# ansonb/RECON

Hardware: AMD Instinct MI355X
Metric: edges aggregated/sec (GAT fwd+bwd) on synthetic KG-context graphs (higher is better)
Workload: dtype f32

## Files before the change

recon_amd/csrc/gat_atp.hip:

```cpp
#include <math.h>
#include <stdlib.h>
#include "recon_common.h"

#include <type_traits>

namespace recon {
namespace {

constexpr int kBlock = 256;

__device__ __forceinline__ int xcd_block(int b, int nb) {
    const int q = nb >> 3, r = nb & 7, x = b & 7, i = b >> 3;
    return (x < r ? x * (q + 1) : r * (q + 1) + (x - r) * q) + i;
}
template <int VEC, bool B16>
__device__ __forceinline__ void load_in(float (&r)[VEC], const float* base, int64_t e) {
    if constexpr (!B16) {
        load_vec<VEC>(r, base + e);
    } else {
        const uint16_t* b = reinterpret_cast<const uint16_t*>(base) + e;
        if constexpr (VEC == 4) {
            const uint2 t = *reinterpret_cast<const uint2*>(b);
            r[0] = __builtin_bit_cast(float, t.x << 16); r[1] = __builtin_bit_cast(float, t.x & 0xffff0000u);
            r[2] = __builtin_bit_cast(float, t.y << 16); r[3] = __builtin_bit_cast(float, t.y & 0xffff0000u);
        } else if constexpr (VEC == 2) {
// ... 70 lines not shown
                                                       const float* __restrict__ gu, int32_t D, int32_t W, float* __restrict__ ga,
                                                       float* __restrict__ ga2, uint32_t* __restrict__ rezero, int32_t rezero_words) {
    __shared__ float red[256];
    const int d = blockIdx.x, h = blockIdx.y;
    if (rezero && d == 0 && h == 0)
        for (int i = threadIdx.x; i < rezero_words; i += 256) rezero[i] = 0u;
    const int64_t row = (static_cast<int64_t>(h) * D + d) * W;
    const float a2v = a2[h * D + d];
    float s = 0.f;
    for (int w = threadIdx.x; w < W; w += 256) {
        const float g = gu[static_cast<int64_t>(h) * W + w];
        s = fmaf(a[row + w], g, s);
        if (ga) ga[row + w] += a2v * g;
    }
    red[threadIdx.x] = s;
    __syncthreads();
    for (int off = 128; off > 0; off >>= 1) {
        if (threadIdx.x < off) red[threadIdx.x] += red[threadIdx.x + off];
        __syncthreads();
    }
    if (threadIdx.x == 0 && ga2) ga2[h * D + d] = red[0];
}

__global__ void __launch_bounds__(256) k_atp_weights_finish(const float* __restrict__ partial, int32_t splits, int32_t W, int32_t D, int32_t H,
                                                            const float* __restrict__ a, const float* __restrict__ a2,
                                                            const float* __restrict__ gu, float* __restrict__ ga, float* __restrict__ ga2,
                                                            uint32_t* __restrict__ rezero, int32_t rezero_words) {
    __shared__ float tile[32][33];
    if (rezero && blockIdx.x == 0)
        for (int i = threadIdx.x; i < rezero_words; i += 256) rezero[i] = 0u;
    const int tw = (W + 31) / 32, td = (D + 31) / 32, ntile = tw * td * H;
    if (static_cast<int>(blockIdx.x) < ntile) {
        const int b = blockIdx.x, h = b / (td * tw), m0 = ((b / td) % tw) * 32, n0 = (b % td) * 32;
        const int tx = threadIdx.x & 31, ty = threadIdx.x >> 5;
        const int64_t MN = static_cast<int64_t>(W) * D;
        const float* pz = partial + static_cast<int64_t>(h) * splits * MN;
        float acc[4] = {0.f, 0.f, 0.f, 0.f};
        int64_t off[4];
        bool ok[4];
#pragma unroll
        for (int i = 0; i < 4; ++i) {
            const int m = m0 + ty + 8 * i, n = n0 + tx;
            ok[i] = m < W && n < D;
            off[i] = ok[i] ? static_cast<int64_t>(m) * D + n : 0;
        }
        for (int z = 0; z < splits; ++z) {
#pragma unroll
            for (int i = 0; i < 4; ++i) acc[i] += pz[z * MN + off[i]];
        }
#pragma unroll
        for (int i = 0; i < 4; ++i) tile[ty + 8 * i][tx] = ok[i] ? acc[i] : 0.f;
        __syncthreads();
#pragma unroll
        for (int i = 0; i < 4; ++i) {
            const int n = n0 + ty + 8 * i, m = m0 + tx;
            if (m < W && n < D)
                ga[(static_cast<int64_t>(h) * D + n) * W + m] = fmaf(a2[h * D + n], gu[static_cast<int64_t>(h) * W + m], tile[tx][ty + 8 * i]);
        }
    } else if (ga2) {
        const int lane = threadIdx.x & 63, wave = threadIdx.x >> 6;
        const int r0 = (static_cast<int>(blockIdx.x) - ntile) * 8 + wave * 2;
#pragma unroll
        for (int i = 0; i < 2; ++i) {
            const int r = r0 + i;
            if (r >= H * D) break;
            const int h = r / D;
            float sum = 0.f;
            for (int w = 4 * lane; w < W; w += 256) {
                const float4 av = *reinterpret_cast<const float4*>(a + static_cast<int64_t>(r) * W + w);
                const float4 gv = *reinterpret_cast<const float4*>(gu + static_cast<int64_t>(h) * W + w);
                sum = fmaf(av.x, gv.x, fmaf(av.y, gv.y, fmaf(av.z, gv.z, fmaf(av.w, gv.w, sum))));
            }
#pragma unroll
            for (int off = 32; off > 0; off >>= 1) sum += __shfl_xor(sum, off, 64);
            if (lane == 0) ga2[r] = sum;
        }
    }
}

__global__ void __launch_bounds__(256) k_elu_grad_q(const float* __restrict__ gy, int32_t ld_gy, const float* __restrict__ y,
// ... 1458 lines not shown
}
template <int NJ, bool B16 = false>
__global__ void __launch_bounds__(256) k_skinny_tn_partial(const SkinnyJob j0, const SkinnyJob j1, const SkinnyJob j2) {
    __shared__ float red[NJ][256];
    const int which = static_cast<int>(blockIdx.x) < j0.nb ? 0 : (static_cast<int>(blockIdx.x) < j0.nb + j1.nb ? 1 : 2);
    const SkinnyJob& jb = which == 0 ? j0 : (which == 1 ? j1 : j2);
    skinny_block<NJ, B16, false>(jb, blockIdx.x - (which == 0 ? 0 : (which == 1 ? j0.nb : j0.nb + j1.nb)), red, nullptr, SkinnySrc{nullptr, nullptr, nullptr}, false);
}

template <int VEC, int KR, bool B16>
__global__ void __launch_bounds__(kBlock) k_gat_atp_src_skinny(const AtpSrcK p, int32_t nsrc, const SkinnyJob j0, const SkinnyJob j1, const SkinnyJob j2,
                                                               const SkinnySrc sr) {
    static_assert(kBlock == 256, "skinny_block: 4 waves");
    __shared__ float red[8][256];
    extern __shared__ __attribute__((aligned(16))) float gsl[];
    const int bx = blockIdx.x;
    if (bx < nsrc) { atp_src_wave<VEC, KR>(p, bx, nsrc); return; }
    const int b = bx - nsrc;
    const int which = b < j0.nb ? 0 : (b < j0.nb + j1.nb ? 1 : 2);
    const SkinnyJob& jb = which == 0 ? j0 : (which == 1 ? j1 : j2);
    skinny_block<8, B16, true>(jb, b - (which == 0 ? 0 : (which == 1 ? j0.nb : j0.nb + j1.nb)), red, gsl, sr, which == 1);
}

struct SkinnyRedJob { const float* partial; float* out; int64_t S1, S2; int32_t nb, nj, K, P, nblocks; };
__global__ void __launch_bounds__(1024) k_skinny_reduce(const SkinnyRedJob j0, const SkinnyRedJob j1, const SkinnyRedJob j2) {
    __shared__ float red[64][17];
    const int which = static_cast<int>(blockIdx.x) < j0.nblocks ? 0 : (static_cast<int>(blockIdx.x) < j0.nblocks + j1.nblocks ? 1 : 2);
    const SkinnyRedJob& jb = which == 0 ? j0 : (which == 1 ? j1 : j2);
    const float* __restrict__ partial = jb.partial;
    float* __restrict__ out = jb.out;
    const int nb = jb.nb, nj = jb.nj, K = jb.K, P = jb.P;
    const int64_t S1 = jb.S1, S2 = jb.S2;
    const int bid = blockIdx.x - (which == 0 ? 0 : (which == 1 ? j0.nblocks : j0.nblocks + j1.nblocks));
    const int e = threadIdx.x & 15, grp = threadIdx.x >> 4;
    const int idx = bid * 16 + e;
    const int tot = nj * K;
    const int per = (nb + 63) / 64;
    const int b0 = grp * per, b1 = min(nb, (grp + 1) * per);
    float s0 = 0.f, s1 = 0.f, s2 = 0.f, s3 = 0.f;
    if (idx < tot) {
        int b = b0;
        for (; b + 4 <= b1; b += 4) {
            s0 += partial[static_cast<int64_t>(b) * tot + idx];
            s1 += partial[static_cast<int64_t>(b + 1) * tot + idx];
            s2 += partial[static_cast<int64_t>(b + 2) * tot + idx];
            s3 += partial[static_cast<int64_t>(b + 3) * tot + idx];
        }
        for (; b < b1; ++b) s0 += partial[static_cast<int64_t>(b) * tot + idx];
    }
    red[grp][e] = (s0 + s1) + (s2 + s3);
    __syncthreads();
    if (grp == 0 && idx < tot) {
        float t = 0.f;
#pragma unroll
        for (int g = 0; g < 64; ++g) t += red[g][e];
        const int j = idx / K, c = idx % K;
        out[(j % P) * S1 + (j / P) * S2 + c] = t;
    }
}

struct AtpShape { int vec, kr, ht; };
bool atp_shape(int F, int R, int H, AtpShape* s) {
    const int mx = F > R ? F : R;
    int vec;
    if (F % 4 == 0 && R % 4 == 0) vec = 4;
    else if (F % 2 == 0 && R % 2 == 0) vec = 2;
    else return false;
    int kr = (mx + 64 * vec - 1) / (64 * vec);
    if (kr > 2 && kr <= 4) kr = 4; else if (kr > 4 && kr <= 8) kr = 8; else if (kr > 8) return false;
    int ht = 1;
    while (ht < H && ht < 8) ht <<= 1;
    while (ht > 1 && 2 * ht * kr * vec > 96) ht >>= 1;
    if (2 * ht * kr * vec > 96) return false;
    s->vec = vec; s->kr = kr; s->ht = ht;
    return true;
}
bool al(const void* p, size_t a) { return (reinterpret_cast<uintptr_t>(p) & (a - 1)) == 0; }
int atp_key(const AtpShape& s) { return s.vec * 1000 + s.kr * 10 + (s.ht == 8 ? 3 : s.ht == 4 ? 2 : s.ht == 2 ? 1 : 0); }

#define ATP_DISPATCH(S, CALL)                                                                              \
    do {                                                                                                   \
// ... 359 lines not shown
    int32_t ld_gh = b->ld_gout;
    const int64_t ld_ghp = bx3_kp(static_cast<int32_t>(HD));
    const bool gh_planes = hx2 || (b->gh_split && a->a_split && !(reinterpret_cast<uintptr_t>(b->gh_split) & 15) && (D % 8) == 0 &&
                                   ((b->ld_gout | a->ld_out) & 3) == 0);
    uint16_t* ghp = gh_planes ? static_cast<uint16_t*>(b->gh_split) : nullptr;
    const int64_t ldi = (static_cast<int64_t>(NR) + 7) / 8 * 8;
    const size_t inv_off = align_up(static_cast<size_t>(2) * N * bx3_kp(static_cast<int32_t>(HD)) * 2, 256);
    const bool row_scaled = hx2 && D <= 256 && ((a->ld_out | b->ld_gout) & 3) == 0 && cfg_char(CFG_ATP_ROW_SCALE) != '0' &&
                            inv_off + static_cast<size_t>(H) * ldi * sizeof(float) <= recon_gat_atp_bwd_split_bytes(N, D, H);
    float* row_inv = row_scaled ? reinterpret_cast<float*>(static_cast<char*>(b->gh_split) + inv_off) : nullptr;
    if (phases & RECON_ATP_BWD_PREPARE) {
        if (hx2 && !row_scaled) {
            rc = hx2_amax(b->grad_out, N, static_cast<int32_t>(HD), b->ld_gout, atp_q(a, 3), st);
            if (rc != RECON_OK) return rc;
        }
        hipLaunchKernelGGL(k_elu_grad_q, dim3(static_cast<unsigned>(ceil_div64(1LL * NR * H, 16))), dim3(256), 0, st, b->grad_out, b->ld_gout, a->out,
                           a->ld_out, NR, H, D, a->concat, ((a->concat || rw.row_node) && !hx2) ? b->g_h : nullptr, b->q, ghp, hx2 ? 2LL * D : ld_ghp,
                           hx2 ? static_cast<int64_t>(D) : static_cast<int64_t>(NR) * ld_ghp, hx2 ? 1 : 0,
                           hx2 ? atp_scale_g(a) : Hx2Scale{nullptr, nullptr, 1.f}, row_inv, ldi, row_scaled ? atp_q(a, 3) : nullptr, rw.row_node);
    }
    if (a->concat || rw.row_node) { gh = b->g_h; ld_gh = static_cast<int32_t>(HD); }
    GemmBatch bt;
    bt.batch = H; bt.epilogue = 0;
    if (phases & RECON_ATP_BWD_INPUTS) {
    {
        OperandDesc A = plain_operand(gh, ld_gh);
        OperandDesc B = plain_operand(a->a, W);
        OutputDesc C = plain_output(b->g_V, static_cast<int64_t>(H) * W);
        bt.a_bs = D; bt.b_bs = static_cast<int64_t>(D) * W; bt.c_bs = W;
        if (hx2)
            rc = gemm_hx2_batched(NR, W, D, b->gh_split, D, 2LL * D, 2LL * NR * D,
                                  static_cast<const char*>(a->a_split) + split_part_bytes(D, W, H), C, bt,
                                  row_scaled ? Hx2Scale{nullptr, nullptr, 1.f} : atp_scale_g(a), atp_scale_a(a), st, 0, row_inv, ldi);
        else if (a->a_split && bx3_supported(A, D, bt))
            rc = gemm_bx3_batched(NR, W, D, A, static_cast<const char*>(a->a_split) + split_part_bytes(D, W, H), C, bt, st);
        else
            rc = gemm_f32_batched(NR, W, D, A, true, B, false, C, bt, 1, nullptr, st);
        if (rc != RECON_OK) return rc;
    }
    {
        AtpBwdK p;
        p.rowptr = rw.rowptr; p.row_node = rw.row_node; p.src = g->src; p.eid = a->ee_index ? a->ee_index : g->eid;
        p.gee_by_slot = a->ee_index ? 1 : 0;
        p.gee_b16 = b->g_ee_bf16 ? 1 : 0;
        if (b->g_ee_bf16 && !(a->io_bf16 && !a->ee_index && b->g_edge_embed && recon_gat_atp_bwd_gee_bf16_supported(F, R, D, H))) return RECON_ERR_UNSUPPORTED;
        p.x = a->x; p.ee = a->edge_embed; p.keep = a->keep; p.sigma = a->sigma; p.Z = a->Z; p.Zk = a->Zk;
// ... 78 lines not shown
                    const Prod& q = pr[i];
                    if (q.rows <= 0) {
                        for (int j = 0; j < q.nj; ++j) (void)hipMemsetAsync(q.out + (j % q.P) * q.S1 + (j / q.P) * q.S2, 0, sizeof(float) * q.K, st);
                        continue;
                    }
                    const int rpb = skinny_rpb(q.rows);
                    const int nb = static_cast<int>(ceil_div64(q.rows, rpb));
                    float* part = b->partial2 + i * third;
                    sj[i] = SkinnyJob{q.G, q.X, q.gather, part, q.ldg, q.nj, q.rows, q.K, rpb, nb};
                    rj[i] = SkinnyRedJob{part, q.out, q.S1, q.S2, nb, q.nj, q.K, q.P, static_cast<int32_t>(ceil_div64(1LL * q.nj * q.K, 16))};
                    if (q.nj > nj_max) nj_max = q.nj;
                    nb_total += nb; nr_total += rj[i].nblocks;
                }
                if (share) { launch_src(); if (nb_total == 0) return; }
                else {
                    if (nb_total == 0) return;
                    const dim3 gp(static_cast<unsigned>(nb_total));
                    if (a->io_bf16) {
                        if (nj_max <= 8) hipLaunchKernelGGL((k_skinny_tn_partial<8, true>), gp, dim3(256), 0, st, sj[0], sj[1], sj[2]);
                        else hipLaunchKernelGGL((k_skinny_tn_partial<16, true>), gp, dim3(256), 0, st, sj[0], sj[1], sj[2]);
                    } else if (nj_max <= 8) hipLaunchKernelGGL((k_skinny_tn_partial<8>), gp, dim3(256), 0, st, sj[0], sj[1], sj[2]);
                    else hipLaunchKernelGGL((k_skinny_tn_partial<16>), gp, dim3(256), 0, st, sj[0], sj[1], sj[2]);
                }
                hipLaunchKernelGGL(k_skinny_reduce, dim3(static_cast<unsigned>(nr_total)), dim3(1024), 0, st, rj[0], rj[1], rj[2]);
            };
            if (H <= 8) {
                const Prod pr[3] = {{b->Gs, 2 * H, H, a->x, rw.row_node, NR, F, H, W, 0, b->g_u},
                                    {b->Gs + H, 2 * H, H, a->x, nullptr, N, F, H, W, 0, b->g_u + F},
                                    {b->g_sigma, H, H, a->edge_embed, ee_gather, E, R, H, W, 0, b->g_u + 2 * F}};
                run_jobs(pr, 3);
            } else {
                for (int j = 0; j < 2 * H; ++j) {
                    const Prod one = {b->Gs + j, 2 * H, 1, a->x, j < H ? rw.row_node : nullptr, j < H ? NR : N, F, 1, W, 0,
                                      b->g_u + static_cast<int64_t>(j % H) * W + (j / H) * F};
                    run_jobs(&one, 1);
                }
                for (int h0 = 0; h0 < H; h0 += 16) {
                    const int nh = H - h0 < 16 ? H - h0 : 16;
                    const Prod one = {b->g_sigma + h0, H, nh, a->edge_embed, ee_gather, E, R, nh, W, 0, b->g_u + static_cast<int64_t>(h0) * W + 2 * F};
                    run_jobs(&one, 1);
                }
            }
        }
        RECON_CHECK_LAUNCH();
    }
    }
    if (b->g_a || b->g_a_2) {
        if (!b->g_a) return RECON_ERR_INVALID;
        if (phases & RECON_ATP_BWD_WEIGHTS) {
            OperandDesc A = plain_operand(a->V, static_cast<int64_t>(H) * W);
            OperandDesc B = plain_operand(gh, ld_gh);
            OutputDesc C = plain_output(b->g_a, W);
            GemmBatch bw = bt;
            bw.a_bs = W; bw.b_bs = D; bw.c_bs = static_cast<int64_t>(D) * W; bw.c_transpose = 1;
            const int64_t ldv = static_cast<int64_t>(H) * W;
            if (hx2) {
                const int sk = bx3_kmajor_splits(NR, bx3_kmajor_split_k(W, D, NR, H));
                rc = gemm_hx2_kmajor_batched(W, D, NR, a->V, 2LL * W, W, 2LL * NR * W, b->gh_split, 2LL * D, D, 2LL * NR * D,
                                             H, sk, b->partial, static_cast<const char*>(a->aux) + kHx2ZeroPageOffset, atp_scale_v(a), atp_scale_g(a), st,
                                             atp_dst_shared(a), row_inv, ldi);
                if (rc == RECON_OK && (phases & RECON_ATP_BWD_EARLY_SUM)) rc = splitk_reduce(b->partial, sk, W, D, C, bw.c_bs, H, 0, true, st);
            } else if (gh_planes && bx3_kmajor_supported(a->V, ldv, W, ld_ghp, D, W, D)) {
                const int sk = bx3_kmajor_splits(NR, bx3_kmajor_split_k(W, D, NR, H));
                rc = gemm_bx3_kmajor_batched(W, D, NR, a->V, ldv, W, b->gh_split, ld_ghp, static_cast<int64_t>(NR) * ld_ghp, D, H, sk, b->partial, st);
                if (rc == RECON_OK) rc = splitk_reduce(b->partial, sk, W, D, C, bw.c_bs, H, 0, true, st);
            } else {
                const int sk = gemm_pick_split_k(W, D, NR, H);
                rc = gemm_f32_batched(W, D, NR, A, false, B, false, C, bw, sk, b->partial, st);
            }
            if (rc != RECON_OK) return rc;
        }
        if ((phases & RECON_ATP_BWD_FINISH) && hx2 && !(phases & RECON_ATP_BWD_EARLY_SUM)) {
            const int sk = bx3_kmajor_splits(NR, bx3_kmajor_split_k(W, D, NR, H));
            const int ntile = static_cast<int>(ceil_div64(W, 32) * ceil_div64(D, 32)) * H;
            hipLaunchKernelGGL(k_atp_weights_finish, dim3(static_cast<unsigned>(ntile + ceil_div64(1LL * H * D, 8))), dim3(256), 0, st, b->partial, sk, W,
                               D, H, a->a, a->a_2, b->g_u, b->g_a, b->g_a_2, atp_q(a, 3), kHx2QuantityWords);
        } else if (phases & RECON_ATP_BWD_FINISH)
        hipLaunchKernelGGL(k_score_vec_bwd, dim3(static_cast<unsigned>(D), static_cast<unsigned>(H)), dim3(256), 0, st, a->a, a->a_2, b->g_u,
                           D, W, b->g_a, b->g_a_2, atp_hx2(a) ? atp_q(a, 3) : nullptr, kHx2QuantityWords);
        RECON_CHECK_LAUNCH();
    } else if ((phases & RECON_ATP_BWD_FINISH) && atp_hx2(a)) {
        if (hipMemsetAsync(atp_q(a, 3), 0, sizeof(uint32_t) * kHx2QuantityWords, st) != hipSuccess) return RECON_ERR_LAUNCH;
    }
    return RECON_OK;
}
```

recon_amd/csrc/gemm_common.h:

```cpp
#pragma once
#include "recon_common.h"

namespace recon {

struct GemmArgs {
    OperandDesc A, B;
    OutputDesc C;
    int32_t M, N, K;
    int32_t k_per_split;
    float* partial;
    int32_t nsplit;
    int32_t epilogue;
    int32_t c_vec4;
    int32_t xcd_remap;
    int64_t a_bs, b_bs, c_bs;
};
enum { GEMM_EPI_NONE = 0, GEMM_EPI_ELU = 1 };

__device__ __forceinline__ float expm1_nonpos(float v) { return __expf(v) - 1.f; }
__device__ __forceinline__ float expm1_nonpos_exact(float v) {
    const float poly = v * fmaf(v, fmaf(v, fmaf(v, 1.f / 24.f, 1.f / 6.f), 0.5f), 1.f);
    return v > -0.0625f ? poly : __expf(v) - 1.f;
}
template <bool EXACT = false>
__device__ __forceinline__ float gemm_epilogue(float v, int epi) {
    if (epi == GEMM_EPI_ELU) return v > 0.f ? v : (EXACT ? expm1_nonpos_exact(v) : expm1_nonpos(v));
    return v;
}

__device__ __forceinline__ int64_t major_off(const OperandDesc& d, int32_t i) {
    if (d.gather) return static_cast<int64_t>(d.gather[i]) * d.S1;
    if (i < d.P) return static_cast<int64_t>(i) * d.S1;
    return static_cast<int64_t>(i % d.P) * d.S1 + static_cast<int64_t>(i / d.P) * d.S2;
}
__device__ __forceinline__ int64_t minor_off(int32_t Dseg, int64_t Sseg, int32_t j) {
    if (j < Dseg) return j;
    return static_cast<int64_t>(j % Dseg) + static_cast<int64_t>(j / Dseg) * Sseg;
}

__device__ __forceinline__ int64_t out_row_off(const OutputDesc& C, int32_t row) {
    if (C.scatter) return static_cast<int64_t>(C.scatter[row]) * C.S1;
    if (row < C.P) return static_cast<int64_t>(row) * C.S1;
    return static_cast<int64_t>(row % C.P) * C.S1 + static_cast<int64_t>(row / C.P) * C.S2;
}

struct TileId { int x, y, z; };
__device__ __forceinline__ TileId xcd_tile(int remap) {
    if (!remap) return {static_cast<int>(blockIdx.x), static_cast<int>(blockIdx.y), static_cast<int>(blockIdx.z)};
    const unsigned gx = gridDim.x, gy = gridDim.y, total = gx * gy * gridDim.z;
    const unsigned L = blockIdx.x + gx * (blockIdx.y + gy * blockIdx.z);
    const unsigned c = L & 7u, pos = L >> 3, q = total >> 3, r = total & 7u;
    const unsigned logical = c * q + min(c, r) + pos;
    TileId id;
    id.x = static_cast<int>(logical % gx);
    const unsigned rest = logical / gx;
    id.y = static_cast<int>(rest % gy);
    id.z = static_cast<int>(rest / gy);
    return id;
}



}
```

recon_amd/csrc/gemm_hx2.hip:

```cpp
#include <stdlib.h>
#include "gemm_tile16.h"

namespace recon {
namespace {

constexpr int T = 2;

struct Hx2Args {
    const _Float16* Ap; const _Float16* Bp;
    int64_t a_plane, a_row, a_bs;
    int64_t b_plane, b_row, b_bs;
    OutputDesc C;
    int64_t c_bs;
    int32_t M, N, K;
    int32_t epilogue, c_vec4, xcd_remap, c_plain;
    int32_t a_shared_k;
    Hx2Scale sa, sb;
    const float* row_inv; int64_t row_inv_bs;
    int32_t a_span_bytes;
};

struct Hx2Terms {
    using V = f16x8;
    static constexpr int T = 2, NP = 3;
// ... 228 lines not shown
    float rsc[2][4];
#pragma unroll
    for (int i = 0; i < 2; ++i)
#pragma unroll
        for (int r = 0; r < 4; ++r)
            rsc[i][r] = (p.row_inv ? p.row_inv[bz * p.row_inv_bs + min(m0 + mb + 16 * i + 4 * lq + r, p.M - 1)] : 1.f) * (ia * ib);
    if (p.c_plain) {
        if (p.epilogue == GEMM_EPI_ELU) hx2_store_plain<GEMM_EPI_ELU>(acc, p.C.base + bz * p.c_bs, p.C.S1, p.M, p.N, m0, n0, mb, li, lq, rsc);
        else hx2_store_plain<GEMM_EPI_NONE>(acc, p.C.base + bz * p.c_bs, p.C.S1, p.M, p.N, m0, n0, mb, li, lq, rsc);
    } else {
        store_permuted<true>(acc, p.C, p.C.base + bz * p.c_bs, p.M, p.N, m0, n0, mb, li, lq, p.epilogue, p.c_vec4, rsc);
    }
}

struct Hx2KmArgs {
    const _Float16* Ap; const _Float16* Bp; const _Float16* zeros;
    int64_t lda, ldb, a_plane, b_plane, a_bs, b_bs;
    float* partial;
    int32_t M, N, K, k_per_split, nsplit;
    int32_t m_ld, n_ld;
    int32_t a_shared_m;
    Hx2Scale sa, sb;
    const float* k_inv; int64_t k_inv_bs;
};

constexpr int KA_PIECES = T * (KA_PLANE / 1024), KA_DMA = KA_PIECES / 4;
constexpr int KB_PIECES = T * (KB_PLANE / 1024), KB_DMA = (KB_PIECES + 3) / 4;

template <int OCC, bool KSC>
__global__ void __launch_bounds__(NT, OCC) k_gemm_hx2_kmajor(const Hx2KmArgs p) {
    __shared__ __attribute__((aligned(16))) unsigned char S[T * KA_PLANE + T * KB_PLANE];
    unsigned char* const As = S;
    unsigned char* const Bs = S + T * KA_PLANE;
    const int t = threadIdx.x, lane = t & 63;
    const int wid = __builtin_amdgcn_readfirstlane(t >> 6);
    const TileId tile = xcd_tile(1);
    const int m0 = tile.y * BM, n0 = tile.x * BN;
    const int bz = tile.z / p.nsplit, zs = tile.z % p.nsplit;
    const int k_begin = zs * p.k_per_split, k_end = min(p.K, k_begin + p.k_per_split);

    int a_k[KA_DMA];
    int64_t a_col[KA_DMA];
#pragma unroll
    for (int i = 0; i < KA_DMA; ++i) {
        const int pc = 4 * i + wid, s = 64 * (pc & 7) + lane, k = s >> 4, phys = s & 15;
        a_k[i] = k;
        a_col[i] = min(m0 + 16 * ((phys >> 1) ^ ka_h(k)) + 8 * (phys & 1), p.m_ld - 8);
        if (a_col[i] >= p.a_shared_m) a_col[i] += bz * p.a_bs;
    }
    int b_k[KB_DMA], b_col[KB_DMA];
#pragma unroll
    for (int i = 0; i < KB_DMA; ++i) {
        const int pc = min(4 * i + wid, KB_PIECES - 1);
        const int s = 64 * (pc % (KB_PIECES / T)) + lane, k = s / KB_SLOTS, phys = s % KB_SLOTS;
        int slot = phys - ((k & 8) ? 2 : 0);
        if (slot < 0 || slot >= 26) slot = 0;
        b_k[i] = k;
        b_col[i] = min(n0 + 8 * slot, p.n_ld - 8);
    }
// ... 240 lines not shown
    if (row_inv && sa.p0) return RECON_ERR_INVALID;
    const bool wide = K >= 1024 && ceil_div64(M, 256) * ceil_div64(N, BN) * bt.batch >= 256;
    const dim3 grid(static_cast<unsigned>(ceil_div64(N, BN)), static_cast<unsigned>(ceil_div64(M, wide ? 256 : BM)), static_cast<unsigned>(bt.batch));
    const int64_t a_span = ((T - 1) * a_plane + (bt.batch - 1) * a_bs + static_cast<int64_t>(M - 1) * a_row + hx2_kp(K) + 8) * 2;
    a.a_span_bytes = (a_plane >= 0 && a_bs >= 0 && a_row >= 0 && a_span < (1LL << 31) - 64) ? static_cast<int32_t>(a_span) : 0;
    const bool ring = !wide && a.a_span_bytes > 0 && cfg_char(CFG_HX2_RING) != '0';
    if (wide) hipLaunchKernelGGL((k_gemm_hx2<8>), grid, dim3(512), 0, st, a);
    else if (ring) hipLaunchKernelGGL((k_gemm_hx2_r3<4>), grid, dim3(NT), 0, st, a);
    else hipLaunchKernelGGL((k_gemm_hx2<4>), grid, dim3(NT), 0, st, a);
    if (hipGetLastError() != hipSuccess) return RECON_ERR_LAUNCH;
    return RECON_OK;
}

bool hx2_kmajor_supported(const void* Ap, int64_t lda, int64_t a_plane, int64_t a_bs, const void* Bp, int64_t ldb, int64_t b_plane,
                          int64_t b_bs, int32_t M, int32_t N) {
    const int64_t m_ld = (static_cast<int64_t>(M) + 7) / 8 * 8, n_ld = (static_cast<int64_t>(N) + 7) / 8 * 8;
    if (M < 1 || N < 1 || ((lda | a_plane | a_bs | ldb | b_plane | b_bs) & 7) || m_ld > lda || n_ld > ldb) return false;
    if (((M & 7) && a_bs != 0) || ((N & 7) && b_bs != 0)) return false;
    return !((reinterpret_cast<uintptr_t>(Ap) | reinterpret_cast<uintptr_t>(Bp)) & 15);
}

int gemm_hx2_kmajor_batched(int32_t M, int32_t N, int32_t K, const void* Ap, int64_t lda, int64_t a_plane, int64_t a_bs, const void* Bp,
                            int64_t ldb, int64_t b_plane, int64_t b_bs, int32_t batch, int32_t split_k, float* partial, const void* zeros,
                            const Hx2Scale& sa, const Hx2Scale& sb, hipStream_t st, int32_t a_shared_m, const float* k_inv, int64_t k_inv_bs) {
    if (M < 0 || N < 0 || K < 0 || batch < 0 || split_k < 1) return RECON_ERR_INVALID;
    if (M == 0 || N == 0 || batch == 0) return RECON_OK;
    if (!Ap || !Bp || !partial || !zeros || (reinterpret_cast<uintptr_t>(zeros) & 15)) return RECON_ERR_INVALID;
    if (!hx2_kmajor_supported(Ap, lda, a_plane, a_bs, Bp, ldb, b_plane, b_bs, M, N)) return RECON_ERR_UNSUPPORTED;
    Hx2KmArgs a;
    a.Ap = static_cast<const _Float16*>(Ap); a.Bp = static_cast<const _Float16*>(Bp); a.zeros = static_cast<const _Float16*>(zeros);
    a.lda = lda; a.ldb = ldb; a.a_plane = a_plane; a.b_plane = b_plane; a.a_bs = a_bs; a.b_bs = b_bs;
    a.partial = partial; a.M = M; a.N = N; a.K = K;
    a.m_ld = (M + 7) / 8 * 8; a.n_ld = (N + 7) / 8 * 8;
    const SplitK sp = splitk_plan(K, split_k);
    a.k_per_split = sp.k_per_split;
    a.nsplit = sp.nsplit;
    if (a.nsplit != split_k) return RECON_ERR_INVALID;
    if (static_cast<int64_t>(batch) * split_k > 65535) return RECON_ERR_UNSUPPORTED;
    a.sa = sa; a.sb = sb;
    if (a_shared_m < 0 || (a_shared_m & 7)) return RECON_ERR_UNSUPPORTED;
    a.a_shared_m = a_shared_m;
    const dim3 grid(static_cast<unsigned>(ceil_div64(N, BN)), static_cast<unsigned>(ceil_div64(M, BM)), static_cast<unsigned>(batch * split_k));
    a.k_inv = k_inv; a.k_inv_bs = k_inv_bs;
    if (k_inv && ((k_inv_bs & 3) || k_inv_bs < ((K + 7) & ~7) || (reinterpret_cast<uintptr_t>(k_inv) & 15))) return RECON_ERR_UNSUPPORTED;
    if (k_inv) hipLaunchKernelGGL((k_gemm_hx2_kmajor<2, true>), grid, dim3(NT), 0, st, a);
    else hipLaunchKernelGGL((k_gemm_hx2_kmajor<2, false>), grid, dim3(NT), 0, st, a);
    if (hipGetLastError() != hipSuccess) return RECON_ERR_LAUNCH;
    return RECON_OK;
}

}

static constexpr size_t kHdr = (recon::kHx2AuxBytes + 255) / 256 * 256;
extern "C" size_t recon_hx2_aux_bytes(void) { return recon::kHx2AuxBytes; }
static size_t hx2_planes_bytes(int64_t rows, int32_t K) { return align_up(static_cast<size_t>(2) * rows * recon::hx2_kp(K) * 2, 256); }

extern "C" size_t recon_sgemm_hx2_workspace_bytes(int32_t M, int32_t N, int32_t K) {
    if (M <= 0 || N <= 0 || K <= 0) return kHdr;
    return kHdr + hx2_planes_bytes(M, K) + hx2_planes_bytes(N, K);
}

extern "C" int recon_sgemm_hx2(int32_t M, int32_t N, int32_t K, const float* A, int32_t lda, const float* B, int32_t ldb, float* C_,
                               int32_t ldc, void* workspace, recon_stream_t stream) {
    using namespace recon;
    if (M < 0 || N < 0 || K < 0) return RECON_ERR_INVALID;
    if (M == 0 || N == 0) return RECON_OK;
    if (!A || !B || !C_ || !workspace || (reinterpret_cast<uintptr_t>(workspace) & 255)) return RECON_ERR_INVALID;
    if (K & 7) return RECON_ERR_UNSUPPORTED;
    hipStream_t st = as_stream(stream);
// ... 78 lines not shown
```

recon_amd/csrc/recon_common.h:

```cpp
#pragma once
#include <hip/hip_runtime.h>
#include <stdint.h>
#include "recon_hip.h"

#define RECON_CHECK_LAUNCH()                                   \
    do {                                                       \
        if (hipGetLastError() != hipSuccess) return RECON_ERR_LAUNCH; \
    } while (0)

static inline hipStream_t as_stream(recon_stream_t s) { return reinterpret_cast<hipStream_t>(s); }
static inline int64_t ceil_div64(int64_t a, int64_t b) { return (a + b - 1) / b; }
static inline size_t align_up(size_t x, size_t a) { return (x + a - 1) / a * a; }

namespace recon {

constexpr int kWave = 64;

enum CfgKey { CFG_GCN_FUSED, CFG_GCN_FUSED_BWD, CFG_GEMM_CFG, CFG_GEMM_LIN, CFG_GEMM_SPLITK, CFG_GEMM_XCD, CFG_PROP_B16, CFG_PROP_B16_YPOST,
              CFG_PROP_BWD, CFG_PROP_BWD_CHAIN, CFG_PROP_BWD_WIDE, CFG_PROP_FWD, CFG_PROP_LDS_KB, CFG_ATP_ROW_SCALE, CFG_GRAPH_SMALL, CFG_KG_NHOP,
              CFG_HX2_RING, CFG_K2_LDS_RING, CFG_K2_PERSIST, CFG_COUNT };
const char* cfg(CfgKey k);
int cfg_int(CfgKey k, int dflt);
char cfg_char(CfgKey k);
int32_t* nan_flag();
// ... 262 lines not shown
        plane = static_cast<int64_t>(p.batch) * R * Cp;
        d = p.dst_n + (static_cast<int64_t>(by) * R + r) * Cp + 8 * kq;
    } else {
        const int c = static_cast<int>(idx % C_), kq = static_cast<int>(idx / C_);
        if (kq >= Rp / 8) return;
#pragma unroll
        for (int j = 0; j < 8; ++j) { const int k = 8 * kq + j; v[j] = k < R ? sp[static_cast<int64_t>(k) * C_ + c] : 0.f; }
        plane = static_cast<int64_t>(p.batch) * C_ * Rp;
        d = p.dst_t + (static_cast<int64_t>(by) * C_ + c) * Rp + 8 * kq;
    }
    uint32_t hi[4], lo[4];
#pragma unroll
    for (int j = 0; j < 4; ++j) hx2_split2(v[2 * j] * s, v[2 * j + 1] * s, hi[j], lo[j]);
    *reinterpret_cast<u32x4_t*>(d) = u32x4_t{hi[0], hi[1], hi[2], hi[3]};
    *reinterpret_cast<u32x4_t*>(d + plane) = u32x4_t{lo[0], lo[1], lo[2], lo[3]};
}
bool hx2_split_both_args(const float* src, int64_t src_bs, int32_t R, int32_t C_, int32_t batch, void* dst_n, void* dst_t, Hx2SplitBoth* p);
int hx2_split_planes_both(const float* src, int64_t src_bs, int32_t R, int32_t C_, int32_t batch, void* dst_n, void* dst_t, const Hx2Scale& sc,
                          hipStream_t st, uint32_t* blkmax_quantity = nullptr, int32_t nblk = 0);
bool hx2_supported(const void* Ap, int64_t a_plane, int64_t a_row, int64_t a_bs, int32_t K);
int gemm_hx2_batched(int32_t M, int32_t N, int32_t K, const void* Ap, int64_t a_plane, int64_t a_row, int64_t a_bs, const void* Bplanes,
                     const OutputDesc& C, const GemmBatch& bt, const Hx2Scale& sa, const Hx2Scale& sb, hipStream_t st, int32_t a_shared_k = 0,
                     const float* row_inv = nullptr, int64_t row_inv_bs = 0);
bool hx2_kmajor_supported(const void* Ap, int64_t lda, int64_t a_plane, int64_t a_bs, const void* Bp, int64_t ldb, int64_t b_plane,
                          int64_t b_bs, int32_t M, int32_t N);
int gemm_hx2_kmajor_batched(int32_t M, int32_t N, int32_t K, const void* Ap, int64_t lda, int64_t a_plane, int64_t a_bs, const void* Bp,
                            int64_t ldb, int64_t b_plane, int64_t b_bs, int32_t batch, int32_t split_k, float* partial, const void* zeros,
                            const Hx2Scale& sa, const Hx2Scale& sb, hipStream_t st, int32_t a_shared_m = 0, const float* k_inv = nullptr,
                            int64_t k_inv_bs = 0);
int splitk_reduce(const float* partial, int32_t splits, int32_t M, int32_t N, const OutputDesc& C, int64_t c_bs, int32_t batch,
                  int32_t epilogue, bool transpose, hipStream_t st);

}
```

Baseline: 81.87 million.

## Fold skinny split-K reduce into kmajor GEMM launch and vectorize weights finish

The skinny split-K reduction is no longer a separate kernel. Its blocks now ride at the front of the hx2 k-major GEMM grid, with the tile index remapped linearly past them, which removes a launch and lets the reduction overlap GEMM tiles. Separately, the weights-finish kernel is rewritten to process 16-row by 256-column strips with float4 partial loads and float4 transposed stores instead of 32x32 scalar tiles, and the host now requires 16-byte alignment. The risks are LDS contention, since riders reuse the GEMM's shared buffer, and fewer finish blocks for small W.

```diff
diff --git a/recon_amd/csrc/gat_atp.hip b/recon_amd/csrc/gat_atp.hip
--- a/recon_amd/csrc/gat_atp.hip
+++ b/recon_amd/csrc/gat_atp.hip
@@ -1,6 +1,7 @@
 #include <math.h>
 #include <stdlib.h>
 #include "recon_common.h"
+#include "skinny_reduce.h"
 
 #include <type_traits>
 
@@ -117,40 +118,58 @@
     if (threadIdx.x == 0 && ga2) ga2[h * D + d] = red[0];
 }
 
+constexpr int kFinishRows = 16, kFinishCols = 256;
 __global__ void __launch_bounds__(256) k_atp_weights_finish(const float* __restrict__ partial, int32_t splits, int32_t W, int32_t D, int32_t H,
                                                             const float* __restrict__ a, const float* __restrict__ a2,
                                                             const float* __restrict__ gu, float* __restrict__ ga, float* __restrict__ ga2,
                                                             uint32_t* __restrict__ rezero, int32_t rezero_words) {
-    __shared__ float tile[32][33];
+    __shared__ __attribute__((aligned(16))) float tile[kFinishRows * (kFinishCols + 4)];
     if (rezero && blockIdx.x == 0)
         for (int i = threadIdx.x; i < rezero_words; i += 256) rezero[i] = 0u;
-    const int tw = (W + 31) / 32, td = (D + 31) / 32, ntile = tw * td * H;
+    const int tw = (W + kFinishRows - 1) / kFinishRows, ntile = tw * H;
     if (static_cast<int>(blockIdx.x) < ntile) {
-        const int b = blockIdx.x, h = b / (td * tw), m0 = ((b / td) % tw) * 32, n0 = (b % td) * 32;
-        const int tx = threadIdx.x & 31, ty = threadIdx.x >> 5;
+        const int t = threadIdx.x, b = blockIdx.x, h = b / tw, w0 = (b % tw) * kFinishRows;
+        const int rows = min(kFinishRows, W - w0);
         const int64_t MN = static_cast<int64_t>(W) * D;
-        const float* pz = partial + static_cast<int64_t>(h) * splits * MN;
-        float acc[4] = {0.f, 0.f, 0.f, 0.f};
-        int64_t off[4];
-        bool ok[4];
-#pragma unroll
-        for (int i = 0; i < 4; ++i) {
-            const int m = m0 + ty + 8 * i, n = n0 + tx;
-            ok[i] = m < W && n < D;
-            off[i] = ok[i] ? static_cast<int64_t>(m) * D + n : 0;
-        }
-        for (int z = 0; z < splits; ++z) {
-#pragma unroll
-            for (int i = 0; i < 4; ++i) acc[i] += pz[z * MN + off[i]];
-        }
-#pragma unroll
-        for (int i = 0; i < 4; ++i) tile[ty + 8 * i][tx] = ok[i] ? acc[i] : 0.f;
-        __syncthreads();
-#pragma unroll
-        for (int i = 0; i < 4; ++i) {
-            const int n = n0 + ty + 8 * i, m = m0 + tx;
-            if (m < W && n < D)
-                ga[(static_cast<int64_t>(h) * D + n) * W + m] = fmaf(a2[h * D + n], gu[static_cast<int64_t>(h) * W + m], tile[tx][ty + 8 * i]);
+        const float* pz = partial + static_cast<int64_t>(h) * splits * MN + static_cast<int64_t>(w0) * D;
+        for (int d0 = 0; d0 < D; d0 += kFinishCols) {
+            const int dc = min(kFinishCols, D - d0), dcq = dc >> 2, ld = dc + 4, nv = rows * dcq;
+            if (d0) __syncthreads();
+            for (int v0 = t; v0 < nv; v0 += 512) {
+                const int v1 = v0 + 256 < nv ? v0 + 256 : v0;
+                const int r0 = v0 / dcq, c0 = 4 * (v0 % dcq), r1 = v1 / dcq, c1 = 4 * (v1 % dcq);
+                const float* p0 = pz + static_cast<int64_t>(r0) * D + d0 + c0;
+                const float* p1 = pz + static_cast<int64_t>(r1) * D + d0 + c1;
+                float4 acc0 = {0.f, 0.f, 0.f, 0.f}, acc1 = {0.f, 0.f, 0.f, 0.f};
+                auto add = [](float4& s, const float4& v) { s.x += v.x; s.y += v.y; s.z += v.z; s.w += v.w; };
+                int z = 0;
+                for (; z + 4 <= splits; z += 4) {
+                    float4 u0[4], u1[4];
+#pragma unroll
+                    for (int i = 0; i < 4; ++i) {
+                        u0[i] = *reinterpret_cast<const float4*>(p0 + (z + i) * MN);
+                        u1[i] = *reinterpret_cast<const float4*>(p1 + (z + i) * MN);
+                    }
+#pragma unroll
+                    for (int i = 0; i < 4; ++i) { add(acc0, u0[i]); add(acc1, u1[i]); }
+                }
+                for (; z < splits; ++z) {
+                    add(acc0, *reinterpret_cast<const float4*>(p0 + z * MN));
+                    add(acc1, *reinterpret_cast<const float4*>(p1 + z * MN));
+                }
+                *reinterpret_cast<float4*>(tile + r0 * ld + c0) = acc0;
+                if (v1 != v0) *reinterpret_cast<float4*>(tile + r1 * ld + c1) = acc1;
+            }
+            __syncthreads();
+            const int nq = rows >> 2;
+            for (int o = t; o < dc * nq; o += 256) {
+                const int wl = 4 * (o % nq), n = d0 + o / nq, m = w0 + wl;
+                const float* tp = tile + wl * ld + (n - d0);
+                const float s = a2[h * D + n];
+                const float4 g = *reinterpret_cast<const float4*>(gu + static_cast<int64_t>(h) * W + m);
+                const float4 r = {fmaf(s, g.x, tp[0]), fmaf(s, g.y, tp[ld]), fmaf(s, g.z, tp[2 * ld]), fmaf(s, g.w, tp[3 * ld])};
+                *reinterpret_cast<float4*>(ga + (static_cast<int64_t>(h) * D + n) * W + m) = r;
+            }
         }
     } else if (ga2) {
         const int lane = threadIdx.x & 63, wave = threadIdx.x >> 6;
@@ -1655,41 +1674,9 @@
     skinny_block<8, B16, true>(jb, b - (which == 0 ? 0 : (which == 1 ? j0.nb : j0.nb + j1.nb)), red, gsl, sr, which == 1);
 }
 
-struct SkinnyRedJob { const float* partial; float* out; int64_t S1, S2; int32_t nb, nj, K, P, nblocks; };
 __global__ void __launch_bounds__(1024) k_skinny_reduce(const SkinnyRedJob j0, const SkinnyRedJob j1, const SkinnyRedJob j2) {
-    __shared__ float red[64][17];
-    const int which = static_cast<int>(blockIdx.x) < j0.nblocks ? 0 : (static_cast<int>(blockIdx.x) < j0.nblocks + j1.nblocks ? 1 : 2);
-    const SkinnyRedJob& jb = which == 0 ? j0 : (which == 1 ? j1 : j2);
-    const float* __restrict__ partial = jb.partial;
-    float* __restrict__ out = jb.out;
-    const int nb = jb.nb, nj = jb.nj, K = jb.K, P = jb.P;
-    const int64_t S1 = jb.S1, S2 = jb.S2;
-    const int bid = blockIdx.x - (which == 0 ? 0 : (which == 1 ? j0.nblocks : j0.nblocks + j1.nblocks));
-    const int e = threadIdx.x & 15, grp = threadIdx.x >> 4;
-    const int idx = bid * 16 + e;
-    const int tot = nj * K;
-    const int per = (nb + 63) / 64;
-    const int b0 = grp * per, b1 = min(nb, (grp + 1) * per);
-    float s0 = 0.f, s1 = 0.f, s2 = 0.f, s3 = 0.f;
-    if (idx < tot) {
-        int b = b0;
-        for (; b + 4 <= b1; b += 4) {
-            s0 += partial[static_cast<int64_t>(b) * tot + idx];
-            s1 += partial[static_cast<int64_t>(b + 1) * tot + idx];
-            s2 += partial[static_cast<int64_t>(b + 2) * tot + idx];
-            s3 += partial[static_cast<int64_t>(b + 3) * tot + idx];
-        }
-        for (; b < b1; ++b) s0 += partial[static_cast<int64_t>(b) * tot + idx];
-    }
-    red[grp][e] = (s0 + s1) + (s2 + s3);
-    __syncthreads();
-    if (grp == 0 && idx < tot) {
-        float t = 0.f;
-#pragma unroll
-        for (int g = 0; g < 64; ++g) t += red[g][e];
-        const int j = idx / K, c = idx % K;
-        out[(j % P) * S1 + (j / P) * S2 + c] = t;
-    }
+    __shared__ float red[kSkinnyRedLdsFloats];
+    skinny_reduce_block<1024>(j0, j1, j2, blockIdx.x, red);
 }
 
 struct AtpShape { int vec, kr, ht; };
@@ -2095,6 +2082,10 @@
     if (a->concat || rw.row_node) { gh = b->g_h; ld_gh = static_cast<int32_t>(HD); }
     GemmBatch bt;
     bt.batch = H; bt.epilogue = 0;
+    const bool ride_ok = hx2 && H <= 8 && b->g_a && (phases & RECON_ATP_BWD_INPUTS) && (phases & RECON_ATP_BWD_WEIGHTS) &&
+                         !(phases & RECON_ATP_BWD_EARLY_SUM);
+    SkinnyRide ride{};
+    bool riding = false;
     if (phases & RECON_ATP_BWD_INPUTS) {
     {
         OperandDesc A = plain_operand(gh, ld_gh);
@@ -2219,7 +2210,8 @@
                     } else if (nj_max <= 8) hipLaunchKernelGGL((k_skinny_tn_partial<8>), gp, dim3(256), 0, st, sj[0], sj[1], sj[2]);
                     else hipLaunchKernelGGL((k_skinny_tn_partial<16>), gp, dim3(256), 0, st, sj[0], sj[1], sj[2]);
                 }
-                hipLaunchKernelGGL(k_skinny_reduce, dim3(static_cast<unsigned>(nr_total)), dim3(1024), 0, st, rj[0], rj[1], rj[2]);
+                if (ride_ok) { ride.j[0] = rj[0]; ride.j[1] = rj[1]; ride.j[2] = rj[2]; riding = true; }
+                else hipLaunchKernelGGL(k_skinny_reduce, dim3(static_cast<unsigned>(nr_total)), dim3(1024), 0, st, rj[0], rj[1], rj[2]);
             };
             if (H <= 8) {
                 const Prod pr[3] = {{b->Gs, 2 * H, H, a->x, rw.row_node, NR, F, H, W, 0, b->g_u},
@@ -2255,7 +2247,7 @@
                 const int sk = bx3_kmajor_splits(NR, bx3_kmajor_split_k(W, D, NR, H));
                 rc = gemm_hx2_kmajor_batched(W, D, NR, a->V, 2LL * W, W, 2LL * NR * W, b->gh_split, 2LL * D, D, 2LL * NR * D,
                                              H, sk, b->partial, static_cast<const char*>(a->aux) + kHx2ZeroPageOffset, atp_scale_v(a), atp_scale_g(a), st,
-                                             atp_dst_shared(a), row_inv, ldi);
+                                             atp_dst_shared(a), row_inv, ldi, riding ? &ride : nullptr);
                 if (rc == RECON_OK && (phases & RECON_ATP_BWD_EARLY_SUM)) rc = splitk_reduce(b->partial, sk, W, D, C, bw.c_bs, H, 0, true, st);
             } else if (gh_planes && bx3_kmajor_supported(a->V, ldv, W, ld_ghp, D, W, D)) {
                 const int sk = bx3_kmajor_splits(NR, bx3_kmajor_split_k(W, D, NR, H));
@@ -2269,7 +2261,8 @@
         }
         if ((phases & RECON_ATP_BWD_FINISH) && hx2 && !(phases & RECON_ATP_BWD_EARLY_SUM)) {
             const int sk = bx3_kmajor_splits(NR, bx3_kmajor_split_k(W, D, NR, H));
-            const int ntile = static_cast<int>(ceil_div64(W, 32) * ceil_div64(D, 32)) * H;
+            const int ntile = static_cast<int>(ceil_div64(W, kFinishRows)) * H;
+            if (!al(b->partial, 16) || !al(b->g_u, 16) || !al(b->g_a, 16)) return RECON_ERR_INVALID;
             hipLaunchKernelGGL(k_atp_weights_finish, dim3(static_cast<unsigned>(ntile + ceil_div64(1LL * H * D, 8))), dim3(256), 0, st, b->partial, sk, W,
                                D, H, a->a, a->a_2, b->g_u, b->g_a, b->g_a_2, atp_q(a, 3), kHx2QuantityWords);
         } else if (phases & RECON_ATP_BWD_FINISH)
diff --git a/recon_amd/csrc/gemm_common.h b/recon_amd/csrc/gemm_common.h
--- a/recon_amd/csrc/gemm_common.h
+++ b/recon_amd/csrc/gemm_common.h
@@ -45,10 +45,7 @@
 }
 
 struct TileId { int x, y, z; };
-__device__ __forceinline__ TileId xcd_tile(int remap) {
-    if (!remap) return {static_cast<int>(blockIdx.x), static_cast<int>(blockIdx.y), static_cast<int>(blockIdx.z)};
-    const unsigned gx = gridDim.x, gy = gridDim.y, total = gx * gy * gridDim.z;
-    const unsigned L = blockIdx.x + gx * (blockIdx.y + gy * blockIdx.z);
+__device__ __forceinline__ TileId xcd_tile_linear(unsigned L, unsigned gx, unsigned gy, unsigned total) {
     const unsigned c = L & 7u, pos = L >> 3, q = total >> 3, r = total & 7u;
     const unsigned logical = c * q + min(c, r) + pos;
     TileId id;
@@ -58,6 +55,11 @@
     id.z = static_cast<int>(rest / gy);
     return id;
 }
+__device__ __forceinline__ TileId xcd_tile(int remap) {
+    if (!remap) return {static_cast<int>(blockIdx.x), static_cast<int>(blockIdx.y), static_cast<int>(blockIdx.z)};
+    const unsigned gx = gridDim.x, gy = gridDim.y;
+    return xcd_tile_linear(blockIdx.x + gx * (blockIdx.y + gy * blockIdx.z), gx, gy, gx * gy * gridDim.z);
+}
 
 
 
diff --git a/recon_amd/csrc/gemm_hx2.hip b/recon_amd/csrc/gemm_hx2.hip
--- a/recon_amd/csrc/gemm_hx2.hip
+++ b/recon_amd/csrc/gemm_hx2.hip
@@ -1,5 +1,6 @@
 #include <stdlib.h>
 #include "gemm_tile16.h"
+#include "skinny_reduce.h"
 
 namespace recon {
 namespace {
@@ -274,19 +275,26 @@
     int32_t a_shared_m;
     Hx2Scale sa, sb;
     const float* k_inv; int64_t k_inv_bs;
+    int32_t gx, gy, ntile;
 };
 
 constexpr int KA_PIECES = T * (KA_PLANE / 1024), KA_DMA = KA_PIECES / 4;
 constexpr int KB_PIECES = T * (KB_PLANE / 1024), KB_DMA = (KB_PIECES + 3) / 4;
 
 template <int OCC, bool KSC>
-__global__ void __launch_bounds__(NT, OCC) k_gemm_hx2_kmajor(const Hx2KmArgs p) {
+__global__ void __launch_bounds__(NT, OCC) k_gemm_hx2_kmajor(const Hx2KmArgs p, const SkinnyRide rd) {
     __shared__ __attribute__((aligned(16))) unsigned char S[T * KA_PLANE + T * KB_PLANE];
+    static_assert(sizeof(S) >= kSkinnyRedLdsFloats * sizeof(float), "the riders' LDS");
+    if (static_cast<int>(blockIdx.x) < rd.nblocks) {
+        if (static_cast<int>(blockIdx.x) < rd.j[0].nblocks + rd.j[1].nblocks + rd.j[2].nblocks)
+            skinny_reduce_block<NT>(rd.j[0], rd.j[1], rd.j[2], blockIdx.x, reinterpret_cast<float*>(S));
+        return;
+    }
     unsigned char* const As = S;
     unsigned char* const Bs = S + T * KA_PLANE;
     const int t = threadIdx.x, lane = t & 63;
     const int wid = __builtin_amdgcn_readfirstlane(t >> 6);
-    const TileId tile = xcd_tile(1);
+    const TileId tile = xcd_tile_linear(blockIdx.x - rd.nblocks, p.gx, p.gy, p.ntile);
     const int m0 = tile.y * BM, n0 = tile.x * BN;
     const int bz = tile.z / p.nsplit, zs = tile.z % p.nsplit;
     const int k_begin = zs * p.k_per_split, k_end = min(p.K, k_begin + p.k_per_split);
@@ -573,9 +581,23 @@
 
 int gemm_hx2_kmajor_batched(int32_t M, int32_t N, int32_t K, const void* Ap, int64_t lda, int64_t a_plane, int64_t a_bs, const void* Bp,
                             int64_t ldb, int64_t b_plane, int64_t b_bs, int32_t batch, int32_t split_k, float* partial, const void* zeros,
-                            const Hx2Scale& sa, const Hx2Scale& sb, hipStream_t st, int32_t a_shared_m, const float* k_inv, int64_t k_inv_bs) {
+                            const Hx2Scale& sa, const Hx2Scale& sb, hipStream_t st, int32_t a_shared_m, const float* k_inv, int64_t k_inv_bs,
+                            const SkinnyRide* ride) {
     if (M < 0 || N < 0 || K < 0 || batch < 0 || split_k < 1) return RECON_ERR_INVALID;
-    if (M == 0 || N == 0 || batch == 0) return RECON_OK;
+    SkinnyRide rd{};
+    if (ride) {
+        rd = *ride;
+        const int64_t nr = static_cast<int64_t>(rd.j[0].nblocks) + rd.j[1].nblocks + rd.j[2].nblocks;
+        if (rd.j[0].nblocks < 0 || rd.j[1].nblocks < 0 || rd.j[2].nblocks < 0 || nr > (1 << 30)) return RECON_ERR_INVALID;
+        rd.nblocks = static_cast<int32_t>((nr + 7) / 8 * 8);
+    }
+    if (M == 0 || N == 0 || batch == 0) {
+        if (rd.nblocks > 0) {
+            hipLaunchKernelGGL((k_gemm_hx2_kmajor<2, false>), dim3(static_cast<unsigned>(rd.nblocks)), dim3(NT), 0, st, Hx2KmArgs{}, rd);
+            if (hipGetLastError() != hipSuccess) return RECON_ERR_LAUNCH;
+        }
+        return RECON_OK;
+    }
     if (!Ap || !Bp || !partial || !zeros || (reinterpret_cast<uintptr_t>(zeros) & 15)) return RECON_ERR_INVALID;
     if (!hx2_kmajor_supported(Ap, lda, a_plane, a_bs, Bp, ldb, b_plane, b_bs, M, N)) return RECON_ERR_UNSUPPORTED;
     Hx2KmArgs a;
@@ -591,11 +613,15 @@
     a.sa = sa; a.sb = sb;
     if (a_shared_m < 0 || (a_shared_m & 7)) return RECON_ERR_UNSUPPORTED;
     a.a_shared_m = a_shared_m;
-    const dim3 grid(static_cast<unsigned>(ceil_div64(N, BN)), static_cast<unsigned>(ceil_div64(M, BM)), static_cast<unsigned>(batch * split_k));
+    a.gx = static_cast<int32_t>(ceil_div64(N, BN)); a.gy = static_cast<int32_t>(ceil_div64(M, BM));
+    const int64_t ntile = static_cast<int64_t>(a.gx) * a.gy * batch * split_k;
+    if (ntile + rd.nblocks >= (1LL << 31)) return RECON_ERR_UNSUPPORTED;
+    a.ntile = static_cast<int32_t>(ntile);
+    const dim3 grid(static_cast<unsigned>(ntile + rd.nblocks));
     a.k_inv = k_inv; a.k_inv_bs = k_inv_bs;
     if (k_inv && ((k_inv_bs & 3) || k_inv_bs < ((K + 7) & ~7) || (reinterpret_cast<uintptr_t>(k_inv) & 15))) return RECON_ERR_UNSUPPORTED;
-    if (k_inv) hipLaunchKernelGGL((k_gemm_hx2_kmajor<2, true>), grid, dim3(NT), 0, st, a);
-    else hipLaunchKernelGGL((k_gemm_hx2_kmajor<2, false>), grid, dim3(NT), 0, st, a);
+    if (k_inv) hipLaunchKernelGGL((k_gemm_hx2_kmajor<2, true>), grid, dim3(NT), 0, st, a, rd);
+    else hipLaunchKernelGGL((k_gemm_hx2_kmajor<2, false>), grid, dim3(NT), 0, st, a, rd);
     if (hipGetLastError() != hipSuccess) return RECON_ERR_LAUNCH;
     return RECON_OK;
 }
diff --git a/recon_amd/csrc/recon_common.h b/recon_amd/csrc/recon_common.h
--- a/recon_amd/csrc/recon_common.h
+++ b/recon_amd/csrc/recon_common.h
@@ -308,12 +308,13 @@
 int gemm_hx2_batched(int32_t M, int32_t N, int32_t K, const void* Ap, int64_t a_plane, int64_t a_row, int64_t a_bs, const void* Bplanes,
                      const OutputDesc& C, const GemmBatch& bt, const Hx2Scale& sa, const Hx2Scale& sb, hipStream_t st, int32_t a_shared_k = 0,
                      const float* row_inv = nullptr, int64_t row_inv_bs = 0);
+struct SkinnyRide;
 bool hx2_kmajor_supported(const void* Ap, int64_t lda, int64_t a_plane, int64_t a_bs, const void* Bp, int64_t ldb, int64_t b_plane,
                           int64_t b_bs, int32_t M, int32_t N);
 int gemm_hx2_kmajor_batched(int32_t M, int32_t N, int32_t K, const void* Ap, int64_t lda, int64_t a_plane, int64_t a_bs, const void* Bp,
                             int64_t ldb, int64_t b_plane, int64_t b_bs, int32_t batch, int32_t split_k, float* partial, const void* zeros,
                             const Hx2Scale& sa, const Hx2Scale& sb, hipStream_t st, int32_t a_shared_m = 0, const float* k_inv = nullptr,
-                            int64_t k_inv_bs = 0);
+                            int64_t k_inv_bs = 0, const SkinnyRide* ride = nullptr);
 int splitk_reduce(const float* partial, int32_t splits, int32_t M, int32_t N, const OutputDesc& C, int64_t c_bs, int32_t batch,
                   int32_t epilogue, bool transpose, hipStream_t st);
 
diff --git a/recon_amd/csrc/skinny_reduce.h b/recon_amd/csrc/skinny_reduce.h
--- /dev/null
+++ b/recon_amd/csrc/skinny_reduce.h
@@ -0,0 +1,76 @@
+#pragma once
+#include <hip/hip_runtime.h>
+#include <stdint.h>
+
+namespace recon {
+
+struct SkinnyRedJob { const float* partial; float* out; int64_t S1, S2; int32_t nb, nj, K, P, nblocks; };
+constexpr int kSkinnyRedLdsFloats = 64 * 17;
+
+struct SkinnyRide { SkinnyRedJob j[3]; int32_t nblocks; };
+
+template <int NTHREADS>
+__device__ __forceinline__ void skinny_reduce_block(const SkinnyRedJob& j0, const SkinnyRedJob& j1, const SkinnyRedJob& j2, int bid_all,
+                                                    float* __restrict__ red) {
+    static_assert(NTHREADS % 16 == 0 && NTHREADS >= 16 && 1024 % NTHREADS == 0, "whole slice groups per pass");
+    const int which = bid_all < j0.nblocks ? 0 : (bid_all < j0.nblocks + j1.nblocks ? 1 : 2);
+    const SkinnyRedJob& jb = which == 0 ? j0 : (which == 1 ? j1 : j2);
+    const float* __restrict__ partial = jb.partial;
+    float* __restrict__ out = jb.out;
+    const int nb = jb.nb, nj = jb.nj, K = jb.K, P = jb.P;
+    const int64_t S1 = jb.S1, S2 = jb.S2;
+    const int bid = bid_all - (which == 0 ? 0 : (which == 1 ? j0.nblocks : j0.nblocks + j1.nblocks));
+    const int e = threadIdx.x & 15;
+    const int idx = bid * 16 + e;
+    const int tot = nj * K;
+    const int per = (nb + 63) / 64;
+    constexpr int G = 1024 / NTHREADS;
+    const int grp0 = threadIdx.x >> 4;
+    int b0[G], nq[G], rem[G];
+    float s[G][4];
+#pragma unroll
+    for (int g = 0; g < G; ++g) {
+        b0[g] = (grp0 + g * (NTHREADS / 16)) * per;
+        const int len = idx < tot ? max(0, min(nb, b0[g] + per) - b0[g]) : 0;
+        nq[g] = len >> 2; rem[g] = len & 3;
+        s[g][0] = s[g][1] = s[g][2] = s[g][3] = 0.f;
+    }
+    for (int k = 0; k < (per >> 2); k += 2) {
+        float v[G][2][4];
+#pragma unroll
+        for (int g = 0; g < G; ++g)
+#pragma unroll
+            for (int u = 0; u < 2; ++u)
+#pragma unroll
+                for (int c = 0; c < 4; ++c)
+                    v[g][u][c] = k + u < nq[g] ? partial[static_cast<int64_t>(b0[g] + 4 * (k + u) + c) * tot + idx] : 0.f;
+#pragma unroll
+        for (int u = 0; u < 2; ++u)
+#pragma unroll
+            for (int g = 0; g < G; ++g)
+                if (k + u < nq[g]) {
+#pragma unroll
+                    for (int c = 0; c < 4; ++c) s[g][c] += v[g][u][c];
+                }
+    }
+#pragma unroll
+    for (int g = 0; g < G; ++g) {
+        float v[3];
+#pragma unroll
+        for (int r = 0; r < 3; ++r) v[r] = r < rem[g] ? partial[static_cast<int64_t>(b0[g] + 4 * nq[g] + r) * tot + idx] : 0.f;
+#pragma unroll
+        for (int r = 0; r < 3; ++r)
+            if (r < rem[g]) s[g][0] += v[r];
+        red[(grp0 + g * (NTHREADS / 16)) * 17 + e] = (s[g][0] + s[g][1]) + (s[g][2] + s[g][3]);
+    }
+    __syncthreads();
+    if (threadIdx.x < 16 && idx < tot) {
+        float t = 0.f;
+#pragma unroll
+        for (int g = 0; g < 64; ++g) t += red[g * 17 + e];
+        const int j = idx / K, c = idx % K;
+        out[(j % P) * S1 + (j / P) * S2 + c] = t;
+    }
+}
+
+}
```

Result: no change. 82.57 million (median of 6 runs) (+0.9%).
